# iamsonderr/icl-mixed-precision-gmres

Hardware: AMD Instinct MI355X
Metric: GMRES iterations/sec + SpMV achieved HBM GB/s, 10M-nnz CSR, 1/2/4/8 GPUs (higher is better)
Workload: dtype f32; 1 GPU; BAND banded CSR n=1000000, offsets -5..+4, nnz=9999975 (1e6 rows = 10M nnz per GPU, 1 GPU(s)); GMRES(30) mixed (fp32 Arnoldi, f32 accumulation, fp64 residual/update), cgs, identity preconditioner, tol=0; step=one restart cycle = 30 iterations, rows_per_gpu=1000000, nnz=9999975, parallelism=one GPU

## Files before the change

icl-mixed-precision-gmres_amd/csrc/arnoldi_kernels.hpp:

```cpp
#pragma once

#include "csr_tile.hpp"
#include "node_tile.hpp"
#include "sell_tile.hpp"
#include "handoff.hpp"
#include "panel.hpp"
#include "internal.hpp"
#include "mpgmres/arnoldi.h"

#include <cstdlib>
#include <new>
#include <algorithm>
#include <vector>

using namespace mpg;

namespace {

constexpr int kNC = 32;
constexpr int kGroups = 1024;
constexpr int kCombineBlock = 1024;
constexpr int kCombineGroups = 256;
constexpr int kOrthMGS = 1, kOrthCGSR = 2;

// ... 780 lines not shown
                                                   const int16_t* __restrict__ col,
                                                   const typename SellStore<VI>::type* __restrict__ val,
                                                   const T* __restrict__ wprev, const T* __restrict__ inv_p,
                                                   T* __restrict__ V, int64_t ld, int k,
                                                   const P* __restrict__ diag, T* __restrict__ w,
                                                   GivensFold<T> fold, SellDots,
                                                   const int32_t* __restrict__ sbase,
                                                   const int32_t* __restrict__ spat, const int64_t* __restrict__ coff, const int16_t* __restrict__ pat,
                                                   const int32_t* __restrict__ xrp,
                                                   const int32_t* __restrict__ xcol,
                                                   const typename SellStore<VI>::type* __restrict__ xval,
                                                   const int8_t* __restrict__ rexp, int64_t ustride, int xcd) {
    using S = typename SellStore<VI>::type;
    using CI = int16_t;
    constexpr bool UNI = true;
    constexpr int SPW = 2;
    constexpr int WL = kWinLen + (SPW - 1) * kWave;
    constexpr int NQ = WL / kWave;
    __shared__ T win[WIN ? BS / kWave : 1][WIN ? WL : 1];
    const int lane = threadIdx.x & (kWave - 1), wid = wave_id();
    const int s0 = ((xcd ? xcd_block(blockIdx.x, gridDim.x) : (int)blockIdx.x) * (BS / kWave) + wid) * SPW;
    const bool live = s0 < nslices;
    bool live_p[SPW];
    const int row0 = s0 * kWave;
    SellRow<S, CI, W, (MPG_SELL_NT != 0), BE> row[SPW];
#pragma unroll
    for (int p = 0; p < SPW; ++p) {
        live_p[p] = s0 + p < nslices;
        const int sp = live_p[p] ? s0 + p : 0;
        if constexpr (UNI) row[p].init_uniform(sp, ustride, spat, coff);
        else row[p].init_load(sp, off, spat, coff);
    }
    __builtin_amdgcn_sched_barrier(0);
    constexpr int NPL = BS < kBlock ? kBlock / BS : 1;
    A part[NPL];
#pragma unroll
    for (int j = 0; j < NPL; ++j) part[j] = A(0);
    if constexpr (FOLD) {
#pragma unroll
        for (int j = 0; j < NPL; ++j) {
            const int t = j * BS + (int)threadIdx.x;
            part[j] = (A)fold.norm2[t < fold.nparts ? t : 0];
            if (t >= fold.nparts) part[j] = A(0);
        }
    }
    __builtin_amdgcn_sched_barrier(0);
    T wr[WIN ? NQ : SPW];
    if constexpr (WIN) {
#pragma unroll
        for (int q = 0; q < NQ; ++q) {
            const int c = row0 - kWinLo + q * kWave + lane;
            wr[q] = wprev[c >= n_lo && c < n_ext ? c : 0];
        }
    } else {
#pragma unroll
        for (int p = 0; p < SPW; ++p) {
            const int i = row0 + p * kWave + lane;
            wr[p] = wprev[i < n ? i : 0];
        }
    }
    __builtin_amdgcn_sched_barrier(0);
    if constexpr (UNI) {
#pragma unroll
        for (int p = 0; p < SPW; ++p) {
            row[p].init_vals(lane, val);
            row[p].load_vals(0);
        }
        __builtin_amdgcn_sched_barrier(0);
#pragma unroll
        for (int p = 0; p < SPW; ++p) {
            row[p].init_finish(lane, col, val, sbase, pat);
            row[p].load_cols(0);
        }
    } else {
#pragma unroll
        for (int p = 0; p < SPW; ++p) {
            row[p].init_finish(lane, col, val, sbase, pat);
            row[p].load(0);
        }
    }
    int rex[SPW] = {};
    if constexpr (std::is_same_v<VI, half_v>) {
        if (rexp) {
#pragma unroll
            for (int p = 0; p < SPW; ++p) {
                const int i = row0 + p * kWave + lane;
                rex[p] = rexp[live_p[p] && i < n ? i : 0];
            }
        }
    }
    __builtin_amdgcn_sched_barrier(0);
    constexpr bool PRE = PG && !WIN;
    using RowT = SellRow<S, CI, W, (MPG_SELL_NT != 0), BE>;
    T xr[PRE ? SPW : 1][PRE ? RowT::U : 1][PRE ? W : 1];
    if constexpr (PRE) {
#pragma unroll
        for (int p = 0; p < SPW; ++p) row[p].gather([&](int c) { return wprev[c]; }, xr[p]);
    }
    __builtin_amdgcn_sched_barrier(0);
    T inv;
    double nrm2sq = 0.0;
    if constexpr (FOLD) {
        constexpr int NG = (BS < kBlock ? kBlock : BS) / kWave;
        __shared__ A scratch[NG];
        __shared__ T inv_s;
        if (fold.nparts > 0) {
#pragma unroll
            for (int j = 0; j < NPL; ++j) {
                const A v = wave_sum(part[j] + A(0));
                if (lane == 0) scratch[j * (BS / kWave) + wid] = v;
            }
            lds_barrier();
            A r = A(0);
#pragma unroll
            for (int q = 0; q < NG; ++q) r += scratch[q];
            nrm2sq = (double)r;
        } else {
            nrm2sq = fold.norm2[0];
        }
        if (threadIdx.x == 0) inv_s = inv_of_norm2<T>(nrm2sq);
        lds_barrier();
        inv = inv_s;
    } else {
        inv = *inv_p;
    }
    if (!live && !(FOLD && blockIdx.x == 0)) return;
    A sum[SPW] = {};
    T vk[SPW] = {};
    if (live) {
        if constexpr (WIN) {
#pragma unroll
            for (int q = 0; q < NQ; ++q) {
                const int c = row0 - kWinLo + q * kWave + lane;
                win[wid][q * kWave + lane] = (c >= n_lo && c < n_ext) ? (T)(wr[q] * inv) : T(0);
            }
            wave_lds_sync();
            auto xv = [&](int c) { return (double)win[wid][c - row0 + kWinLo]; };
#pragma unroll
            for (int p = 0; p < SPW; ++p) row[p].sum(0, xv, sum[p]);
#pragma unroll
            for (int p = 0; p < SPW; ++p) {
                for (int q = row[p].U; q < row[p].steps; q += row[p].U) {
                    row[p].load(q);
                    row[p].sum(q, xv, sum[p]);
                }
                vk[p] = win[wid][p * kWave + lane + kWinLo];
            }
        } else {
            auto xv = [&](int c) { return (double)(T)(wprev[c] * inv); };
#pragma unroll
            for (int p = 0; p < SPW; ++p) {
                const int i = row0 + p * kWave + lane;
                if (SellCol<CI>::stepped && row[p].exc) {
                    sum[p] = csr_row_sum<A>(live_p[p] && i < n ? row[p].xrow : -1, xrp, xcol, xval, xv);
                } else {
                    if constexpr (PRE) row[p].sum_gathered(0, xr[p], [&](T r) { return (double)(T)(r * inv); }, sum[p]);
                    else row[p].sum(0, xv, sum[p]);
                    for (int q = row[p].U; q < row[p].steps; q += row[p].U) {
                        row[p].load(q);
                        row[p].sum(q, xv, sum[p]);
                    }
                }
                vk[p] = (T)(wr[p] * inv);
            }
        }
    }
#pragma unroll
    for (int p = 0; p < SPW; ++p) {
        const int i = row0 + p * kWave + lane;
        if (live_p[p] && i < n) {
            double sp = sum[p];
            if constexpr (std::is_same_v<VI, half_v>) sp = ldexp(sp, -rex[p]);
            const T t = (T)sp;
            w[i] = precond<T, P>(t, diag, i);
            V[(int64_t)k * ld + i] = vk[p];
        }
    }
    if constexpr (FOLD) {
        __shared__ T col_s[kFoldMaxM + 2], c_s[kFoldMaxM + 2], s_s[kFoldMaxM + 2];
        if (blockIdx.x == 0) givens_block(fold.g, nrm2sq, col_s, c_s, s_s);
    }
}

template <class T, int BS = kBlock, bool COMBINE = false, class A = double>
__global__ __launch_bounds__(BS) void k_panel_dots(int n, const T* __restrict__ V, int64_t ld, int c0, int nc,
                                                   const T* __restrict__ w, double* __restrict__ partial,
                                                   unsigned* __restrict__ cnt, double* __restrict__ sums) {
    A acc[kNC];
#pragma unroll
    for (int c = 0; c < kNC; ++c) acc[c] = A(0);
    const int n4 = n & ~3;
    const T* __restrict__ Vb = V + (int64_t)c0 * ld;
    for (int i = 4 * (blockIdx.x * BS + threadIdx.x); i < n4; i += 4 * gridDim.x * BS) {
        A wv[4];
        Row4<T>::load(w + i, wv);
#pragma unroll
        for (int c = 0; c < kNC; ++c) {
            if (c < nc) {
                A v[4];
                Row4<T>::load(Vb + (int64_t)c * ld + i, v);
                acc[c] += v[0] * wv[0] + v[1] * wv[1] + v[2] * wv[2] + v[3] * wv[3];
            }
        }
    }
    for (int i = n4 + blockIdx.x * BS + threadIdx.x; i < n; i += gridDim.x * BS) {
        const A wi = (A)w[i];
#pragma unroll
        for (int c = 0; c < kNC; ++c)
            if (c < nc) acc[c] += (A)Vb[(int64_t)c * ld + i] * wi;
    }
    store_partials<kNC, BS, COMBINE>(acc, nc, partial + (size_t)c0 * gridDim.x);
    if constexpr (COMBINE) {
        if (last_arriver(cnt)) combine_columns<BS, A>(partial, gridDim.x, nc, sums);
    }
}

template <class T, class A>
struct DotsGlobal {
    static constexpr bool kStaged = false;
    static constexpr int kHeld = 0;
    const T* __restrict__ w;
    Raw4<T> held[1];
    __device__ __forceinline__ void load_w(int i, A (&wv)[4]) const { Row4<T>::load(w + i, wv); }
    __device__ __forceinline__ Raw4<T> newest(int) const { return Raw4<T>(); }
};

template <class T, int BS, int NC, class A = double, class SRC>
__device__ __forceinline__ void dots_panel_from(int n, const T* __restrict__ V, int64_t ld, const SRC& src,
                                           double* __restrict__ partial) {
    static_assert(NC >= 1 && NC <= kNC, "one panel");
    constexpr int NP = Pow2Ceil<NC>::v;
    constexpr int B = kColBatch<T>;
    A acc[NP];
#pragma unroll
    for (int c = 0; c < NP; ++c) acc[c] = A(0);
    const int n4 = n & ~3;
    bool first = SRC::kHeld > 0;
    for (int i = 4 * (blockIdx.x * BS + threadIdx.x); i < n4; i += 4 * gridDim.x * BS) {
        A wv[4];
        src.load_w(i, wv);
#pragma unroll
        for (int c0 = 0; c0 < NC; c0 += B) {
            Raw4<T> v[B];
#pragma unroll
            for (int u = 0; u < B; ++u)
                if (c0 + u < NC) {
                    if (SRC::kStaged && c0 + u == NC - 1) v[u] = src.newest(i);
                    else if (c0 + u < SRC::kHeld && first) v[u] = src.held[c0 + u < SRC::kHeld ? c0 + u : 0];
                    else v[u].load(V + (int64_t)(c0 + u) * ld + i);
                }
            __builtin_amdgcn_sched_barrier(0);
#pragma unroll
            for (int u = 0; u < B; ++u)
                if (c0 + u < NC)
                    acc[c0 + u] += v[u].template at<A>(0) * wv[0] + v[u].template at<A>(1) * wv[1] +
                                   v[u].template at<A>(2) * wv[2] + v[u].template at<A>(3) * wv[3];
            asm volatile("" : "+v"(acc[c0]) : : "memory");
        }
        if constexpr (SRC::kHeld > 0) first = false;
    }
    if constexpr (!SRC::kStaged) {
        for (int i = n4 + blockIdx.x * BS + threadIdx.x; i < n; i += gridDim.x * BS) {
            const A wi = (A)src.w[i];
#pragma unroll
            for (int c = 0; c < NC; ++c) acc[c] += (A)V[(int64_t)c * ld + i] * wi;
        }
    }
    store_partials<NP, BS>(acc, NC, partial);
}

template <class T, int BS, int NC, class A = double>
__device__ __forceinline__ void dots_panel(int n, const T* __restrict__ V, int64_t ld, const T* __restrict__ w,
                                           double* __restrict__ partial) {
    dots_panel_from<T, BS, NC, A>(n, V, ld, DotsGlobal<T, A>{w, {}}, partial);
}

template <class T, int BS, int NC, bool STAMP = false, class A = double>
__global__ __launch_bounds__(BS) void k_dots_nc(int n, const T* __restrict__ V, int64_t ld,
                                                const T* __restrict__ w, double* __restrict__ partial,
                                                unsigned long long* stamp) {
    stamp_at<STAMP>(stamp, 0);
    dots_panel<T, BS, NC, A>(n, V, ld, w, partial);
    stamp_at<STAMP>(stamp, 1);
}

constexpr int kStepDotsRows = 4 * kCombineBlock;

template <class T, class A, int HELD>
struct DotsStaged {
    static constexpr bool kStaged = true;
    static constexpr int kHeld = HELD;
    const T* wst;
    const T* vkst;
    int base;
    Raw4<T> held[HELD > 0 ? HELD : 1];
    __device__ __forceinline__ void load_w(int i, A (&wv)[4]) const { Row4<T>::load(wst + (i - base), wv); }
    __device__ __forceinline__ Raw4<T> newest(int i) const {
        Raw4<T> r;
        r.load(vkst + (i - base));
        return r;
    }
};

template <class T, class P, int W, bool FOLD, int BE, int NC, bool PF, class A>
__global__ __launch_bounds__(kCombineBlock) void k_step_dots(int n, int nslices, const int16_t* __restrict__ col,
                                                             const T* __restrict__ val, const T* __restrict__ wprev,
                                                             const T* __restrict__ inv_p, T* __restrict__ V,
                                                             int64_t ld, int k, const P* __restrict__ diag,
                                                             T* __restrict__ w, GivensFold<T> fold,
                                                             const int32_t* __restrict__ spat,
                                                             const int64_t* __restrict__ coff,
                                                             const int16_t* __restrict__ pat, int64_t ustride,
                                                             double* __restrict__ dpart) {
    static_assert(std::is_same_v<T, float>, "fp32 basis and values");
    using CI = int16_t;
    using Row = SellRow<T, CI, W, (MPG_SELL_NT != 0), BE>;
    constexpr int BS = kCombineBlock, SPW = 4;
    constexpr int RB = kStepDotsRows, WL = kWinLo + RB + kWinHi;
    static_assert(SPW * (BS / kWave) * kWave == RB, "four slices per wave cover the workgroup's rows");
    __shared__ __attribute__((aligned(16))) T win[WL];
    __shared__ __attribute__((aligned(16))) T wst[RB];
    const int tid = threadIdx.x, lane = tid & (kWave - 1), wid = wave_id();
    const int base = (int)blockIdx.x * RB;
    const int s0 = (int)blockIdx.x * (RB / kWave) + wid * SPW;
    Row row[SPW];
    bool live_p[SPW];
#pragma unroll
    for (int p = 0; p < SPW; ++p) {
        live_p[p] = s0 + p < nslices;
        row[p].init_uniform(live_p[p] ? s0 + p : 0, ustride, spat, coff);
    }
    __builtin_amdgcn_sched_barrier(0);
    A part = A(0);
    if constexpr (FOLD) {
        part = (A)fold.norm2[tid < fold.nparts ? tid : 0];
        if (tid >= fold.nparts) part = A(0);
    }
    __builtin_amdgcn_sched_barrier(0);
    const int i4 = base + 4 * tid;
    const bool in4 = i4 < n;
    Raw4<T> wr;
    wr.load(wprev + (in4 ? i4 : 0));
    const int hc = tid < kWinLo ? base - kWinLo + tid : base + RB + (tid - kWinLo);
    const bool hin = tid < kWinLo + kWinHi && hc >= 0 && hc < n;
    const T wh = wprev[hin ? hc : 0];
    __builtin_amdgcn_sched_barrier(0);
#pragma unroll
    for (int p = 0; p < SPW; ++p) {
        row[p].init_vals(lane, val);
        row[p].load_vals(0);
    }
    __builtin_amdgcn_sched_barrier(0);
#pragma unroll
    for (int p = 0; p < SPW; ++p) {
        row[p].init_finish(lane, col, val, nullptr, pat);
        row[p].load_cols(0);
    }
    __builtin_amdgcn_sched_barrier(0);
    constexpr int B = kColBatch<T>;
    constexpr int HMAX = FOLD ? 6 : B;
    constexpr int HELD = !PF ? 0 : NC - 1 < HMAX ? NC - 1 : HMAX;
    DotsStaged<T, A, HELD> src;
    src.wst = wst;
    src.vkst = win + kWinLo;
    src.base = base;
    if constexpr (HELD > 0) {
#pragma unroll
        for (int u = 0; u < HELD; ++u) src.held[u].load(V + (int64_t)u * ld + (in4 ? i4 : 0));
    }
    __builtin_amdgcn_sched_barrier(0);
    T inv;
    double nrm2sq = 0.0;
    if constexpr (FOLD) {
        constexpr int NG = kBlock / kWave;
        __shared__ A scratch[NG];
        __shared__ T inv_s;
        if (fold.nparts > 0) {
            if (wid < NG) {
                const A v = wave_sum(part + A(0));
                if (lane == 0) scratch[wid] = v;
            }
            lds_barrier();
            A r = A(0);
#pragma unroll
            for (int q = 0; q < NG; ++q) r += scratch[q];
            nrm2sq = (double)r;
        } else {
            nrm2sq = fold.norm2[0];
        }
        if (tid == 0) inv_s = inv_of_norm2<T>(nrm2sq);
        lds_barrier();
        inv = inv_s;
    } else {
        inv = *inv_p;
    }
    {
        T vq[4];
#pragma unroll
        for (int r = 0; r < 4; ++r) vq[r] = in4 ? (T)(wr.template at<T>(r) * inv) : T(0);
        Row4<T>::store(win + kWinLo + 4 * tid, vq);
        if (tid < kWinLo + kWinHi) win[tid < kWinLo ? tid : RB + tid] = hin ? (T)(wh * inv) : T(0);
    }
    lds_barrier();
    auto xv = [&](int c) { return (double)win[c - base + kWinLo]; };
    A sum[SPW] = {};
#pragma unroll
    for (int p = 0; p < SPW; ++p)
        if (live_p[p]) row[p].sum(0, xv, sum[p]);
#pragma unroll
    for (int p = 0; p < SPW; ++p) {
        if (live_p[p])
            for (int q = Row::U; q < row[p].steps; q += Row::U) {
                row[p].load(q);
                row[p].sum(q, xv, sum[p]);
            }
        const int i = (s0 + p) * kWave + lane;
        T wi = T(0);
        if (live_p[p] && i < n) {
            const T t = (T)sum[p];
            wi = precond<T, P>(t, diag, i);
            w[i] = wi;
            V[(int64_t)k * ld + i] = win[i - base + kWinLo];
        }
        wst[i - base] = wi;
    }
    lds_barrier();
    dots_panel_from<T, BS, NC, A>(n, V, ld, src, dpart);
    if constexpr (FOLD) {
        __shared__ T col_s[kFoldMaxM + 2], c_s[kFoldMaxM + 2], s_s[kFoldMaxM + 2];
        if (blockIdx.x == 0) givens_block(fold.g, nrm2sq, col_s, c_s, s_s);
    }
}

template <class T, int BS, int NCL, class A = double>
__global__ __launch_bounds__(BS) void k_dots_panels(int n, const T* __restrict__ V, int64_t ld,
                                                    const T* __restrict__ w, double* __restrict__ partial) {
    const int c0 = blockIdx.y * kNC;
    double* __restrict__ part = partial + (size_t)c0 * gridDim.x;
    if (blockIdx.y + 1 < gridDim.y) dots_panel<T, BS, kNC, A>(n, V + (int64_t)c0 * ld, ld, w, part);
    else dots_panel<T, BS, NCL, A>(n, V + (int64_t)c0 * ld, ld, w, part);
}

template <class T, int BS, int NC, bool FROM_PARTS = false, bool NEXT_DOTS = false, bool PF = false,
          bool STAMP = false, class A = double>
__global__ __launch_bounds__(BS) void k_cgs_update_nc(int n, const T* __restrict__ V, int64_t ld,
                                                      const double* __restrict__ sums, int part_G,
                                                      T* __restrict__ coef_out, T* __restrict__ w,
                                                      double* __restrict__ partial, unsigned long long* stamp) {
    static_assert(NC >= 1 && NC <= kNC, "one panel");
    stamp_at<STAMP>(stamp, 0);
    static_assert(!FROM_PARTS || BS >= 32 * NC, "32 lanes per column");
    static_assert(!PF || (FROM_PARTS && !NEXT_DOTS), "prefetch under the partial sums");
    static_assert(!PF || NC <= kColBatch<T>, "the prefetch form holds one batch of columns (the only form run)");
    constexpr int B = kColBatch<T>;
    constexpr int B0 = NC < B ? NC : B;
    __shared__ A coef[NC];
    const int n4 = n & ~3;
    const int i_first = 4 * (blockIdx.x * BS + threadIdx.x);
    Raw4<T> pw, pv[PF ? B0 : 1];
    if constexpr (FROM_PARTS) {
        const int j = threadIdx.x / 32, sub = threadIdx.x % 32;
        const int jc = j < NC ? j : NC - 1;
        constexpr int Q = kCombineGroups / 32;
        A pp[Q];
#pragma unroll
        for (int q = 0; q < Q; ++q) {
            const int g = sub + 32 * q;
            pp[q] = (A)sums[(size_t)jc * part_G + (g < part_G ? g : 0)];
        }
        if constexpr (PF) {
            __builtin_amdgcn_sched_barrier(0);
            const int ip = i_first < n4 ? i_first : 0;
            pw.load(w + ip);
#pragma unroll
            for (int u = 0; u < B0; ++u) pv[u].load(V + (int64_t)u * ld + ip);
            __builtin_amdgcn_sched_barrier(0);
        }
        A v = A(0);
#pragma unroll
        for (int q = 0; q < Q; ++q)
            if (sub + 32 * q < part_G) v += pp[q];
#pragma unroll
        for (int o = 16; o > 0; o >>= 1) v += __shfl_xor(v, o, kWave);
        if (j < NC && sub == 0) {
            const T c = (T)v;
            coef[j] = (A)c;
            if (blockIdx.x == 0) coef_out[j] = c;
        }
    } else if (threadIdx.x < NC) {
        const T c = (T)sums[threadIdx.x];
        coef[threadIdx.x] = (A)c;
        if (blockIdx.x == 0) coef_out[threadIdx.x] = c;
    }
    if constexpr (PF) lds_barrier();
    else __syncthreads();
    constexpr int NA = NEXT_DOTS ? Pow2Ceil<NC>::v : 1;
    A acc[NA];
#pragma unroll
    for (int c = 0; c < NA; ++c) acc[c] = A(0);
    bool first = PF;
    for (int i = i_first; i < n4; i += 4 * gridDim.x * BS) {
        Raw4<T> wr;
        if (first) wr = pw;
        else wr.load(w + i);
        A t[4] = {A(0), A(0), A(0), A(0)};
#pragma unroll
        for (int c0 = 0; c0 < NC; c0 += B) {
            Raw4<T> v[B];
#pragma unroll
            for (int u = 0; u < B; ++u)
                if (c0 + u < NC) {
                    if (c0 == 0 && first) v[u] = pv[u < B0 ? u : 0];
                    else v[u].load(V + (int64_t)(c0 + u) * ld + i);
                }
            __builtin_amdgcn_sched_barrier(0);
#pragma unroll
            for (int u = 0; u < B; ++u)
                if (c0 + u < NC) {
                    const A cu = coef[c0 + u];
#pragma unroll
                    for (int r = 0; r < 4; ++r) t[r] += v[u].template at<A>(r) * cu;
                }
        }
        T wo[4];
        A wd[4];
#pragma unroll
        for (int r = 0; r < 4; ++r) {
            wo[r] = T(-1) * (T)t[r] + T(1) * (T)wr[r];
            wd[r] = (A)wo[r];
            if (!NEXT_DOTS) acc[0] += wd[r] * wd[r];
        }
        Row4<T>::store(w + i, wo);
        first = false;
        if constexpr (NEXT_DOTS) {
#pragma unroll
            for (int c0 = 0; c0 < NC; c0 += B) {
                Raw4<T> v[B];
#pragma unroll
                for (int u = 0; u < B; ++u)
                    if (c0 + u < NC) v[u].load(V + (int64_t)(c0 + u) * ld + i);
                __builtin_amdgcn_sched_barrier(0);
#pragma unroll
                for (int u = 0; u < B; ++u)
                    if (c0 + u < NC)
                        acc[c0 + u] += v[u].template at<A>(0) * wd[0] + v[u].template at<A>(1) * wd[1] +
                                       v[u].template at<A>(2) * wd[2] + v[u].template at<A>(3) * wd[3];
            }
        }
    }
    for (int i = n4 + blockIdx.x * BS + threadIdx.x; i < n; i += gridDim.x * BS) {
        A t = A(0);
#pragma unroll
        for (int j = 0; j < NC; ++j) t += (A)V[(int64_t)j * ld + i] * coef[j];
        const T wi = T(-1) * (T)t + T(1) * w[i];
        w[i] = wi;
        if constexpr (NEXT_DOTS) {
#pragma unroll
            for (int c = 0; c < NC; ++c) acc[c] += (A)V[(int64_t)c * ld + i] * (A)wi;
        } else {
            acc[0] += (A)wi * (A)wi;
        }
    }
    store_partials<NA, BS>(acc, NEXT_DOTS ? NC : 1, partial);
    stamp_at<STAMP>(stamp, 1);
}

constexpr int kWideMax = 128;
template <class T, int BS, class A = double>
__global__ __launch_bounds__(BS) void k_cgs_update_wide(int n, const T* __restrict__ V, int64_t ld, int nc,
                                                        const double* __restrict__ parts, int part_G,
                                                        T* __restrict__ coef_out, T* __restrict__ w,
                                                        double* __restrict__ partial) {
    constexpr int LPC = BS / kWideMax, Q = 128 / LPC, B = kColBatch<T>;
    static_assert(LPC * kWideMax == BS && Q * LPC == 128, "8 lanes per column, <= 128 partials");
    __shared__ A coef[kWideMax];
    {
        const int j = threadIdx.x / LPC, sub = threadIdx.x % LPC;
        const int jc = j < nc ? j : nc - 1;
        A pp[Q];
#pragma unroll
        for (int q = 0; q < Q; ++q) {
            const int g = sub + LPC * q;
            pp[q] = (A)parts[(size_t)jc * part_G + (g < part_G ? g : 0)];
        }
        A v = A(0);
#pragma unroll
        for (int q = 0; q < Q; ++q)
            if (sub + LPC * q < part_G) v += pp[q];
#pragma unroll
        for (int o = LPC / 2; o > 0; o >>= 1) v += __shfl_xor(v, o, kWave);
        if (sub == 0) {
            const T c = (T)v;
            coef[j] = j < nc ? (A)c : A(0);
            if (blockIdx.x == 0 && j < nc) coef_out[j] = c;
        }
    }
    __syncthreads();
    A acc[1] = {A(0)};
    const int n4 = n & ~3;
    const int nb = (nc + B - 1) / B;
    for (int i = 4 * (blockIdx.x * BS + threadIdx.x); i < n4; i += 4 * gridDim.x * BS) {
        Raw4<T> wr;
        wr.load(w + i);
        A t[4] = {A(0), A(0), A(0), A(0)};
        for (int bi = 0; bi < nb; ++bi) {
            const int c0 = bi * B;
            Raw4<T> v[B];
#pragma unroll
            for (int u = 0; u < B; ++u) {
                const int c = c0 + u < nc ? c0 + u : nc - 1;
                v[u].load(V + (int64_t)c * ld + i);
            }
            __builtin_amdgcn_sched_barrier(0);
#pragma unroll
            for (int u = 0; u < B; ++u) {
                const A cu = coef[c0 + u < kWideMax ? c0 + u : kWideMax - 1];
                if (c0 + u < nc)
#pragma unroll
                    for (int r = 0; r < 4; ++r) t[r] += v[u].template at<A>(r) * cu;
            }
        }
        T wo[4];
#pragma unroll
        for (int r = 0; r < 4; ++r) {
            wo[r] = T(-1) * (T)t[r] + T(1) * (T)wr[r];
            const A wd = (A)wo[r];
            acc[0] += wd * wd;
        }
        Row4<T>::store(w + i, wo);
    }
    for (int i = n4 + blockIdx.x * BS + threadIdx.x; i < n; i += gridDim.x * BS) {
        A t = A(0);
        for (int j = 0; j < nc; ++j) t += (A)V[(int64_t)j * ld + i] * coef[j];
        const T wi = T(-1) * (T)t + T(1) * w[i];
        w[i] = wi;
        acc[0] += (A)wi * (A)wi;
    }
    store_partials<1, BS>(acc, 1, partial);
}

template <int N, class F>
int with_nc(int nc, F&& f) {
    if constexpr (N == 0) {
        return MPG_ERR_ARG;
    } else {
        if (nc == N) return f(std::integral_constant<int, N>());
        return with_nc<N - 1>(nc, f);
    }
}

template <class T, bool NEXT_DOTS, bool GIVENS = false, int BS = kBlock, bool FROM_PARTS = false, class A = double>
__global__ __launch_bounds__(BS) void k_cgs_update(int n, const T* __restrict__ V, int64_t ld, int k,
                                                       const double* __restrict__ sums, T* __restrict__ coef_out,
                                                       T* __restrict__ w, double* __restrict__ partial,
                                                       unsigned* __restrict__ cnt, GivensArgs<T> g, int part_G) {
    static_assert(!(NEXT_DOTS && GIVENS), "the Givens step follows the last pass");
    __shared__ A coef[256];
    const int nc = k + 1;
    const int n4 = n & ~3;
    const int i_first = 4 * (blockIdx.x * BS + threadIdx.x);
    constexpr int kPre = 8;
    const int npre = nc < kPre ? nc : kPre;
    const bool pre = FROM_PARTS && i_first < n4;
    A pv[kPre][4], pw[4];
    if (pre) {
#pragma unroll
        for (int u = 0; u < kPre; ++u)
            if (u < npre) Row4<T>::load(V + (int64_t)u * ld + i_first, pv[u]);
        Row4<T>::load(w + i_first, pw);
    }
    if (FROM_PARTS) {
        constexpr int LPC = BS / kNC;
        const int j = threadIdx.x / LPC, sub = threadIdx.x % LPC;
        const int per = (part_G + LPC - 1) / LPC;
        A v = A(0);
        if (j < nc) {
            const double* src = sums + (size_t)j * part_G + sub;
#pragma unroll 8
            for (int q = 0; q < per; ++q)
                if (q * LPC + sub < part_G) v += (A)src[q * LPC];
        }
#pragma unroll
        for (int o = LPC / 2; o > 0; o >>= 1) v += __shfl_xor(v, o, kWave);
        if (j < nc && sub == 0) {
            const T c = (T)v;
            coef[j] = (A)c;
            if (blockIdx.x == 0) coef_out[j] = c;
        }
    } else {
        for (int j = threadIdx.x; j < nc; j += BS) {
            const T c = (T)sums[j];
            coef[j] = (A)c;
            if (blockIdx.x == 0) coef_out[j] = c;
        }
    }
    __syncthreads();
    constexpr int NA = NEXT_DOTS ? kNC : 1;
    A acc[NA];
#pragma unroll
    for (int c = 0; c < NA; ++c) acc[c] = A(0);
    for (int i = i_first; i < n4; i += 4 * gridDim.x * BS) {
        A t[4] = {A(0), A(0), A(0), A(0)};
        int j = 0;
        const bool use_pre = pre && i == i_first;
        if (use_pre) {
#pragma unroll
            for (int u = 0; u < kPre; ++u)
                if (u < npre)
#pragma unroll
                    for (int r = 0; r < 4; ++r) t[r] += pv[u][r] * coef[u];
            j = npre;
        }
        for (; j + 8 <= nc; j += 8) {
            A v[8][4];
#pragma unroll
            for (int u = 0; u < 8; ++u) Row4<T>::load(V + (int64_t)(j + u) * ld + i, v[u]);
#pragma unroll
            for (int u = 0; u < 8; ++u)
#pragma unroll
                for (int r = 0; r < 4; ++r) t[r] += v[u][r] * coef[j + u];
        }
        for (; j < nc; ++j) {
            A v[4];
            Row4<T>::load(V + (int64_t)j * ld + i, v);
#pragma unroll
            for (int r = 0; r < 4; ++r) t[r] += v[r] * coef[j];
        }
        A wv[4];
        if (use_pre) {
// ... 391 lines not shown
```

Baseline: 27360 GMRES iterations/s.

## Replace workgroup barriers in step-dots kernel with per-wave LDS windows and handoffs

Gives each wave its own halo window in LDS so it stages only its own rows plus halo and synchronises with a wave-local handoff instead of workgroup barriers. The norm reduction for the fold path is now done redundantly in every wave via wave sums and readfirstlane, which removes the shared scratch and two more barriers. The aim is to let waves of the 1024-thread block proceed independently through SpMV and the dot panel. In exchange, each wave loads its own halo, so halo reads are duplicated, LDS use grows, and every wave repeats the reduction work.

Measured after the change: 28970 GMRES iterations/s (median of 6 runs). 5.9% higher.

```diff
diff --git a/icl-mixed-precision-gmres_amd/csrc/arnoldi_kernels.hpp b/icl-mixed-precision-gmres_amd/csrc/arnoldi_kernels.hpp
--- a/icl-mixed-precision-gmres_amd/csrc/arnoldi_kernels.hpp
+++ b/icl-mixed-precision-gmres_amd/csrc/arnoldi_kernels.hpp
@@ -1106,6 +1106,21 @@
     }
 };
 
+__device__ __forceinline__ void wave_lds_handoff() {
+    __atomic_signal_fence(__ATOMIC_SEQ_CST);
+    __builtin_amdgcn_s_waitcnt(0xC07F);
+    wave_lds_sync();
+    __atomic_signal_fence(__ATOMIC_SEQ_CST);
+}
+
+__device__ __forceinline__ float wave_first(float v) {
+    return __int_as_float(__builtin_amdgcn_readfirstlane(__float_as_int(v)));
+}
+__device__ __forceinline__ double wave_first(double v) {
+    return __hiloint2double(__builtin_amdgcn_readfirstlane(__double2hiint(v)),
+                            __builtin_amdgcn_readfirstlane(__double2loint(v)));
+}
+
 template <class T, class P, int W, bool FOLD, int BE, int NC, bool PF, class A>
 __global__ __launch_bounds__(kCombineBlock) void k_step_dots(int n, int nslices, const int16_t* __restrict__ col,
                                                              const T* __restrict__ val, const T* __restrict__ wprev,
@@ -1119,13 +1134,16 @@
     static_assert(std::is_same_v<T, float>, "fp32 basis and values");
     using CI = int16_t;
     using Row = SellRow<T, CI, W, (MPG_SELL_NT != 0), BE>;
-    constexpr int BS = kCombineBlock, SPW = 4;
-    constexpr int RB = kStepDotsRows, WL = kWinLo + RB + kWinHi;
-    static_assert(SPW * (BS / kWave) * kWave == RB, "four slices per wave cover the workgroup's rows");
-    __shared__ __attribute__((aligned(16))) T win[WL];
+    constexpr int BS = kCombineBlock, SPW = 4, NW = BS / kWave;
+    constexpr int RB = kStepDotsRows, RW = SPW * kWave;
+    constexpr int WL = kWinLo + RW + kWinHi;
+    static_assert(NW * RW == RB, "four slices per wave cover the workgroup's rows");
+    static_assert(RW == 4 * kWave, "a wave's slices are its lanes' row groups of dots_panel_from");
+    __shared__ __attribute__((aligned(16))) T win[NW][WL];
     __shared__ __attribute__((aligned(16))) T wst[RB];
     const int tid = threadIdx.x, lane = tid & (kWave - 1), wid = wave_id();
     const int base = (int)blockIdx.x * RB;
+    const int row0 = base + wid * RW;
     const int s0 = (int)blockIdx.x * (RB / kWave) + wid * SPW;
     Row row[SPW];
     bool live_p[SPW];
@@ -1135,19 +1153,25 @@
         row[p].init_uniform(live_p[p] ? s0 + p : 0, ustride, spat, coff);
     }
     __builtin_amdgcn_sched_barrier(0);
-    A part = A(0);
+    constexpr int NG = kBlock / kWave;
+    A part[NG];
     if constexpr (FOLD) {
-        part = (A)fold.norm2[tid < fold.nparts ? tid : 0];
-        if (tid >= fold.nparts) part = A(0);
+#pragma unroll
+        for (int q = 0; q < NG; ++q) {
+            const int t = q * kWave + lane;
+            part[q] = (A)fold.norm2[t < fold.nparts ? t : 0];
+            if (t >= fold.nparts) part[q] = A(0);
+        }
     }
     __builtin_amdgcn_sched_barrier(0);
     const int i4 = base + 4 * tid;
     const bool in4 = i4 < n;
     Raw4<T> wr;
     wr.load(wprev + (in4 ? i4 : 0));
-    const int hc = tid < kWinLo ? base - kWinLo + tid : base + RB + (tid - kWinLo);
-    const bool hin = tid < kWinLo + kWinHi && hc >= 0 && hc < n;
-    const T wh = wprev[hin ? hc : 0];
+    const int clo = row0 - kWinLo + lane, chi = row0 + RW + lane;
+    const bool lo_in = clo >= 0 && clo < n, hi_in = chi < n;
+    const T wlo = wprev[lo_in ? clo : 0];
+    const T whi = wprev[hi_in ? chi : 0];
     __builtin_amdgcn_sched_barrier(0);
 #pragma unroll
     for (int p = 0; p < SPW; ++p) {
@@ -1164,10 +1188,11 @@
     constexpr int B = kColBatch<T>;
     constexpr int HMAX = FOLD ? 6 : B;
     constexpr int HELD = !PF ? 0 : NC - 1 < HMAX ? NC - 1 : HMAX;
+    T* const wwin = win[wid];
     DotsStaged<T, A, HELD> src;
-    src.wst = wst;
-    src.vkst = win + kWinLo;
-    src.base = base;
+    src.wst = wst + wid * RW;
+    src.vkst = wwin + kWinLo;
+    src.base = row0;
     if constexpr (HELD > 0) {
 #pragma unroll
         for (int u = 0; u < HELD; ++u) src.held[u].load(V + (int64_t)u * ld + (in4 ? i4 : 0));
@@ -1176,25 +1201,15 @@
     T inv;
     double nrm2sq = 0.0;
     if constexpr (FOLD) {
-        constexpr int NG = kBlock / kWave;
-        __shared__ A scratch[NG];
-        __shared__ T inv_s;
         if (fold.nparts > 0) {
-            if (wid < NG) {
-                const A v = wave_sum(part + A(0));
-                if (lane == 0) scratch[wid] = v;
-            }
-            lds_barrier();
             A r = A(0);
 #pragma unroll
-            for (int q = 0; q < NG; ++q) r += scratch[q];
+            for (int q = 0; q < NG; ++q) r += wave_first(wave_sum(part[q] + A(0)));
             nrm2sq = (double)r;
         } else {
             nrm2sq = fold.norm2[0];
         }
-        if (tid == 0) inv_s = inv_of_norm2<T>(nrm2sq);
-        lds_barrier();
-        inv = inv_s;
+        inv = inv_of_norm2<T>(nrm2sq);
     } else {
         inv = *inv_p;
     }
@@ -1202,11 +1217,12 @@
         T vq[4];
 #pragma unroll
         for (int r = 0; r < 4; ++r) vq[r] = in4 ? (T)(wr.template at<T>(r) * inv) : T(0);
-        Row4<T>::store(win + kWinLo + 4 * tid, vq);
-        if (tid < kWinLo + kWinHi) win[tid < kWinLo ? tid : RB + tid] = hin ? (T)(wh * inv) : T(0);
-    }
-    lds_barrier();
-    auto xv = [&](int c) { return (double)win[c - base + kWinLo]; };
+        Row4<T>::store(wwin + kWinLo + 4 * lane, vq);
+        wwin[lane] = lo_in ? (T)(wlo * inv) : T(0);
+        wwin[kWinLo + RW + lane] = hi_in ? (T)(whi * inv) : T(0);
+    }
+    wave_lds_handoff();
+    auto xv = [&](int c) { return (double)wwin[c - row0 + kWinLo]; };
     A sum[SPW] = {};
 #pragma unroll
     for (int p = 0; p < SPW; ++p)
@@ -1224,11 +1240,11 @@
             const T t = (T)sum[p];
             wi = precond<T, P>(t, diag, i);
             w[i] = wi;
-            V[(int64_t)k * ld + i] = win[i - base + kWinLo];
+            V[(int64_t)k * ld + i] = wwin[i - row0 + kWinLo];
         }
         wst[i - base] = wi;
     }
-    lds_barrier();
+    wave_lds_handoff();
     dots_panel_from<T, BS, NC, A>(n, V, ld, src, dpart);
     if constexpr (FOLD) {
         __shared__ T col_s[kFoldMaxM + 2], c_s[kFoldMaxM + 2], s_s[kFoldMaxM + 2];
```
